# JakobHavtorn/benchmarking-lvms

Hardware: AMD Instinct MI355X
Metric: audio frames/sec training (VRNN, 16 kHz mu-law) (higher is better)
Workload: dtype f32

## Files before the change

### benchmarking-lvms_amd/csrc/pchain.h

```cpp
#pragma once
#include <algorithm>
#include <cstdlib>

#include "common.h"

namespace blvm {
namespace pchain {

constexpr unsigned SENTINEL = 0xFFFFFFFFu;
constexpr unsigned SPIN_LIMIT = 1u << 22;

typedef unsigned u32x4 __attribute__((ext_vector_type(4)));
typedef __amdgpu_buffer_rsrc_t rsrc_t;
constexpr int AUX_SC1 = 16;
#ifndef PCHAIN_POLL_AUX
#define PCHAIN_POLL_AUX AUX_SC1
#endif
#ifndef PCHAIN_STORE_AUX
#define PCHAIN_STORE_AUX AUX_SC1
#endif
__device__ __forceinline__ rsrc_t make_rsrc(const void* base) {
  const unsigned long long u = reinterpret_cast<unsigned long long>(base);
  const unsigned lo = (unsigned)__builtin_amdgcn_readfirstlane((int)(unsigned)u), hi = (unsigned)__builtin_amdgcn_readfirstlane((int)(unsigned)(u >> 32));
  return __builtin_amdgcn_make_buffer_rsrc(reinterpret_cast<void*>(((unsigned long long)hi << 32) | lo), 0, 0xFFFFFFFFu, 0x00020000);
}
__device__ __forceinline__ f32x4 ld_sc1_x4(rsrc_t r, unsigned byte_off) {
  return __builtin_bit_cast(f32x4, __builtin_amdgcn_raw_buffer_load_b128(r, (int)byte_off, 0, PCHAIN_POLL_AUX));
}
__device__ __forceinline__ float ld_sc1(rsrc_t r, unsigned byte_off) {
  return __builtin_bit_cast(float, __builtin_amdgcn_raw_buffer_load_b32(r, (int)byte_off, 0, PCHAIN_POLL_AUX));
}
__device__ __forceinline__ void st_sc1(rsrc_t r, unsigned byte_off, float v) {
  __builtin_amdgcn_raw_buffer_store_b32(__builtin_bit_cast(unsigned, v), r, (int)byte_off, 0, PCHAIN_STORE_AUX);
}

__device__ __forceinline__ bool is_sentinel(float x) { return __float_as_uint(x) == SENTINEL; }
__device__ __forceinline__ bool any_sentinel(const f32x4& v) {
  return is_sentinel(v[0]) | is_sentinel(v[1]) | is_sentinel(v[2]) | is_sentinel(v[3]);
}

struct Ctl {
  unsigned* dev;
  unsigned* host;
  unsigned epoch;
  __device__ __forceinline__ bool aborted() const { return __hip_atomic_load(dev, __ATOMIC_RELAXED, __HIP_MEMORY_SCOPE_AGENT) == epoch; }
  __device__ __forceinline__ void abort(unsigned code) const {
    if (__hip_atomic_exchange(dev, epoch, __ATOMIC_RELAXED, __HIP_MEMORY_SCOPE_AGENT) != epoch) {
      __hip_atomic_store(host + 1, code, __ATOMIC_RELAXED, __HIP_MEMORY_SCOPE_SYSTEM);
      __hip_atomic_fetch_add(host, 1u, __ATOMIC_RELAXED, __HIP_MEMORY_SCOPE_SYSTEM);
    }
  }
};

__device__ __forceinline__ bool spin_tick(unsigned& spins, const Ctl& ctl, unsigned code, bool& dead) {
  ++spins;
  if ((spins & 255u) == 0) {
    if (ctl.aborted()) { dead = true; return true; }
    if (spins >= SPIN_LIMIT) { ctl.abort(code); dead = true; return true; }
  }
  return false;
}

struct Poll {
  Ctl ctl;
  unsigned code;
  bool dead;
  int nap;
#ifdef PCHAIN_TPROF
  unsigned long long t_first = 0, t_ok = 0, t_end = 0, tp[8] = {0, 0, 0, 0, 0, 0, 0, 0};
  unsigned polls = 0;
#endif
  __device__ __forceinline__ void sleep() const {
    if (nap > 8) __builtin_amdgcn_s_sleep(32);
    else __builtin_amdgcn_s_sleep(1);
  }
};

struct MapSame { static constexpr int of(int) { return 0; } static constexpr bool sum = false; };
struct MapId { static constexpr int of(int g) { return g; } static constexpr bool sum = false; };
struct MapPairs { static constexpr int of(int g) { return g >> 1; } static constexpr bool sum = false; };
struct MapSum { static constexpr int of(int) { return 0; } static constexpr bool sum = true; };

struct NoMid {
  __device__ __forceinline__ void operator()() const {}
};

typedef short s16x4 __attribute__((ext_vector_type(4)));
typedef unsigned u32x2 __attribute__((ext_vector_type(2)));
typedef float f32x2_t __attribute__((ext_vector_type(2)));
typedef __bf16 bf16x2_t __attribute__((ext_vector_type(2)));
typedef _Float16 f16x2_t __attribute__((ext_vector_type(2)));
typedef _Float16 f16x4_t __attribute__((ext_vector_type(4)));
__device__ __forceinline__ unsigned pk_bf16(float a, float b) {
  return __builtin_bit_cast(unsigned, __builtin_convertvector((f32x2_t){a, b}, bf16x2_t));
}
template <int OT>
__device__ __forceinline__ unsigned pk16(float a, float b) {
  if constexpr (OT == OP_F16) return __builtin_bit_cast(unsigned, __builtin_convertvector((f32x2_t){a, b}, f16x2_t));
  else return pk_bf16(a, b);
}
template <int OT>
__device__ __forceinline__ f32x4 mfma16(s16x4 a, s16x4 b, f32x4 acc) {
  if constexpr (OT == OP_F16)
    return __builtin_amdgcn_mfma_f32_16x16x16f16(__builtin_bit_cast(f16x4_t, a), __builtin_bit_cast(f16x4_t, b), acc, 0, 0, 0);
  else return __builtin_amdgcn_mfma_f32_16x16x16bf16_1k(a, b, acc, 0, 0, 0);
}
template <int OT> struct WFrag { typedef u32x2 type; };
template <> struct WFrag<OP_F32> { typedef f32x4 type; };

template <int NW, int OT, int GA, int G, class AMap, int CH, class Mid>
__device__ __forceinline__ void mgemm_trip(const rsrc_t (&ar)[GA], unsigned aoff, const float* const (&ap)[GA], const char* const (&wp)[G], int kc,
                                           bool aok, bool polled, f32x4 (&acc)[G], Poll& pl, Mid& mid, bool& mid_pending) {
  constexpr int STEP = NW * 16;
  typedef typename WFrag<OT>::type wfrag;
  constexpr int ES = OT != OP_F32 ? 2 : 4;
  wfrag w[G][CH];
  f32x4 a[GA][CH];
#pragma unroll
  for (int u = 0; u < CH; ++u)
#pragma unroll
    for (int g = 0; g < G; ++g) w[g][u] = *reinterpret_cast<const wfrag*>(wp[g] + (size_t)ES * 16 * (size_t)(kc + u * STEP));
  if (!polled) {
#pragma unroll
// ... 303 lines not shown
  LinLate L;
  auto prefetch = [&]() {
    L = late();
    if (L.bias) e_bias = L.bias[col];
    if (L.gate) e_gate = L.gate[(size_t)rowc * L.ldgate + col];
    if (L.add && !L.add_polled) e_add = L.add[(size_t)rowc * L.ldadd + col];
  };
  f32x4 acc[1] = {{0.f, 0.f, 0.f, 0.f}};
  if (A2 != nullptr) {
    const float* const As[3] = {A, A2, A3};
    const float* const Ws[1] = {W};
    const int la[3] = {0, 0, 0}, cs[1] = {c0};
    tile_product<NW, OT, 3, 1, MapSum>(ws, As, la, true, r0, B, Ws, cs, K, acc, pl, prefetch, lda, w_width);
  } else {
    const float* const As[1] = {A};
    const float* const Ws[1] = {W};
    const int la[1] = {lda}, cs[1] = {c0};
    tile_product<NW, OT, 1, 1, MapSame>(ws, As, la, a_polled, r0, B, Ws, cs, K, acc, pl, prefetch, a_polled ? lda : 0, w_width);
  }
  float v[1];
  reduce_tiles<1, NW>(acc, red, v);
#ifdef PCHAIN_TPROF
  if (a_polled && pl.nap == 1) {
    const unsigned long long t3 = wall_clock64();
    pl.tp[0] += 1; pl.tp[1] += pl.t_first - t0; pl.tp[2] += pl.t_ok - pl.t_first; pl.tp[3] += t3 - pl.t_ok; pl.tp[4] += pl.polls;
    if (pl.t_end != 0) pl.tp[6] += t0 - pl.t_end;
  }
#endif
  if (threadIdx.x >= 256) return;
  if (L.add && L.add_polled) {
    const rsrc_t rs[1] = {make_rsrc(L.add)};
    const unsigned os[1] = {4u * ((unsigned)rowc * (unsigned)L.ldadd + (unsigned)col)};
    float ws[1];
    poll_words<1>(rs, os, ws, own, pl);
    e_add = ws[0];
  }
  if (!own) return;
  float x = v[0] + e_bias + e_add;
  if (L.relu) x = x > 0.f ? x : x * L.slope;
  if (L.gate) x = e_gate > 0.f ? x : x * L.slope;
  put(L.out, r0, c0, row, col, x);
#ifdef PCHAIN_TPROF
  if (a_polled && pl.nap == 1) { pl.t_end = wall_clock64(); }
#endif
}
template <int NW, int OT = OP_F32>
__device__ __forceinline__ void tile_lin(const float* A, int lda, bool a_polled, const float* W, int K, const float* bias,
                                         const float* add, int ldadd, bool add_polled, const float* gate, int ldgate, bool relu,
                                         float slope, const Out& out, int r0, int c0, int B, float* red, Poll& pl) {
  auto late = [&]() { return LinLate{bias, add, gate, ldadd, ldgate, add_polled, relu, slope, out}; };
  tile_lin_late<NW, OT>(A, lda, a_polled, W, K, late, r0, c0, B, red, pl);
}

struct HeadOut {
  float *mu_p, *sd_p, *mu_q, *sd_q, *raw_p, *raw_q, *muq_raw;
  Out z;
};
template <int NW, int OT = OP_F32, class WS = WMem>
__device__ __forceinline__ void tile_head(const float* P, const float* Q, bool polled, const float* Wp, const float* bp, const float* Wq,
                                          const float* bq, const float* eps, const HeadOut& o, int H, int Z, int residual, float beta,
                                          float inv_beta, float sd_eps, int r0, int c0, int B, float* red, Poll& pl, const WS& ws = WS()) {
  const int t = threadIdx.x & 255;
  const int row = r0 + (t >> 4), col = c0 + (t & 15);
  const bool own = threadIdx.x < 256 && row < B;
  const size_t oc = (size_t)(row < B ? row : r0) * Z + col;
  float b0 = 0.f, b1 = 0.f, b2 = 0.f, b3 = 0.f, e = 0.f;
  auto prefetch = [&]() { b0 = bp[col]; b1 = bp[Z + col]; b2 = bq[col]; b3 = bq[Z + col]; e = eps[oc]; };
  f32x4 acc[4];
#pragma unroll
  for (int g = 0; g < 4; ++g) acc[g] = (f32x4){0.f, 0.f, 0.f, 0.f};
  {
    const float* const As[2] = {P, Q};
    const float* const Ws[4] = {Wp, Wp, Wq, Wq};
    const int la[2] = {H, H}, cs[4] = {c0, Z + c0, c0, Z + c0};
    tile_product<NW, OT, 2, 4, MapPairs>(ws, As, la, polled, r0, B, Ws, cs, H, acc, pl, prefetch);
  }
  float v[4];
  reduce_tiles<4, NW>(acc, red, v);
  if (!own) return;
  const size_t oo = (size_t)row * Z + col;
  const float mp = v[0] + b0, rp = v[1] + b1, rq = v[3] + b3;
  float mq = v[2] + b2;
  const float sp = softplus_beta(rp, beta, inv_beta) + sd_eps;
  const float sq = softplus_beta(rq, beta, inv_beta) + sd_eps;
  if (o.muq_raw != nullptr) o.muq_raw[oo] = mq;
  float sqc = sq;
  if (residual == 1) {
    mq += mp;
  } else if (residual == 2) {
    const float pq = 1.f / (sq * sq), pp = 1.f / (sp * sp);
    const float var = 1.f / (pq + pp);
    mq = var * (mq * pq + mp * pp);
    sqc = sqrtf(var);
  } else if (residual == 3) {
    mq = mp;
    sqc = sp;
  }
  put(o.z, r0, c0, row, col, e * sqc + mq);
  o.mu_p[oo] = mp; o.sd_p[oo] = sp; o.mu_q[oo] = mq; o.sd_q[oo] = sqc;
  o.raw_p[oo] = rp; o.raw_q[oo] = rq;
}

template <int NW, int OT = OP_F32, class WS = WMem>
__device__ __forceinline__ void tile_gru(const float* X, int ldx, bool polled, const float* Wih, int K, const float* xg, const float* bih,
                                         const float* gh, const float* hprev, int ldh, int R, const Out& hnew, float* rg, float* ug, float* ng,
                                         int r0, int c0, int B, float* red, Poll& pl, const WS& ws = WS()) {
  const int t = threadIdx.x & 255;
  const int row = r0 + (t >> 4), col = c0 + (t & 15);
  const bool own = threadIdx.x < 256 && row < B;
  const int rowc = row < B ? row : r0;
  const size_t o3 = (size_t)rowc * 3 * R + col;
  const rsrc_t rgh = make_rsrc(gh), rhp = make_rsrc(hprev);
  const rsrc_t ps[4] = {rgh, rgh, rgh, rhp};
  const unsigned po[4] = {4u * (unsigned)o3, 4u * (unsigned)(o3 + R), 4u * (unsigned)(o3 + 2 * R), 4u * ((unsigned)rowc * (unsigned)ldh + (unsigned)col)};
  float w[4] = {0.f, 0.f, 0.f, 0.f}, x0 = 0.f, x1 = 0.f, x2 = 0.f;
  auto prefetch = [&]() {
#pragma unroll
    for (int i = 0; i < 4; ++i) w[i] = ld_sc1(ps[i], po[i]);
    x0 = (xg ? xg[o3] : 0.f) + (bih ? bih[col] : 0.f);
    x1 = (xg ? xg[o3 + R] : 0.f) + (bih ? bih[R + col] : 0.f);
    x2 = (xg ? xg[o3 + 2 * R] : 0.f) + (bih ? bih[2 * R + col] : 0.f);
  };
  f32x4 acc[3];
#pragma unroll
  for (int g = 0; g < 3; ++g) acc[g] = (f32x4){0.f, 0.f, 0.f, 0.f};
  {
    const float* const As[1] = {X};
    const float* const Ws[3] = {Wih, Wih, Wih};
    const int la[1] = {ldx}, cs[3] = {c0, R + c0, 2 * R + c0};
    tile_product<NW, OT, 1, 3, MapSame>(ws, As, la, polled, r0, B, Ws, cs, K, acc, pl, prefetch);
  }
  float v[3];
  reduce_tiles<3, NW>(acc, red, v);
  if (threadIdx.x >= 256) return;
  if (__any(own && (is_sentinel(w[0]) | is_sentinel(w[1]) | is_sentinel(w[2]) | is_sentinel(w[3])))) poll_words<4>(ps, po, w, own, pl);
  if (!own) return;
  const float r = sigmoidf_(v[0] + x0 + w[0]);
  const float u = sigmoidf_(v[1] + x1 + w[1]);
  const float n = tanhf(v[2] + x2 + r * w[2]);
  put(hnew, r0, c0, row, col, (1.f - u) * n + u * w[3]);
  const size_t o = (size_t)row * R + col;
  rg[o] = r; ug[o] = u; ng[o] = n;
}

struct DzIn {
  const float *mu_q, *sd_q, *mu_p, *sd_p, *eps, *raw_q, *raw_p, *muq_raw;
  const int32_t* x_sl;
  const float *c_raw, *c_fn;
  int t, stride, residual;
  float fn_floor, beta, sd_eps;
  bool has_gemm = true;
};
template <int NW, int OT = OP_F32, class WS = WMem>
__device__ __forceinline__ void tile_dz(const float* D, const float* WT, const float* D2, const float* WT2, bool polled, const float* dz_add,
                                        int ld_add, bool add_polled, const DzIn& a, const Out& dqh, const Out& dph, int H, int Z, int r0, int c0,
                                        int B, float* red, Poll& pl, const WS& ws = WS()) {
  const int t = threadIdx.x & 255;
  const int row = r0 + (t >> 4), col = c0 + (t & 15);
  const bool own = threadIdx.x < 256 && row < B;
  const int rowc = row < B ? row : r0;
  const size_t o = (size_t)rowc * Z + col;
  float mq = 0.f, sq = 1.f, mp = 0.f, sp = 1.f, e = 0.f, rq = 0.f, rp = 0.f, c_raw = 0.f, c_fn = 0.f, e_add = 0.f;
  auto prefetch = [&]() {
    mq = a.mu_q[o]; sq = a.sd_q[o]; mp = a.mu_p[o]; sp = a.sd_p[o]; e = a.eps[o]; rq = a.raw_q[o]; rp = a.raw_p[o];
    if (a.c_fn != nullptr || a.c_raw != nullptr) {
      const bool live = (long long)a.t * a.stride < a.x_sl[rowc];
      c_raw = (live && a.c_raw != nullptr) ? a.c_raw[rowc] : 0.f;
      c_fn = (live && a.c_fn != nullptr) ? a.c_fn[rowc] : 0.f;
    }
    if (dz_add != nullptr && !add_polled) e_add = dz_add[(size_t)rowc * ld_add + col];
  };
  float v[2] = {0.f, 0.f};
  if (a.has_gemm) {
    f32x4 acc[2];
    acc[0] = (f32x4){0.f, 0.f, 0.f, 0.f};
    acc[1] = (f32x4){0.f, 0.f, 0.f, 0.f};
    if (WS::products != 1 && D2 != nullptr) {
      if constexpr (WS::products != 1) {
        const float* const As[2] = {D, D2};
        const float* const Ws[2] = {WT, WT2};
        const int la[2] = {H, H}, cs[2] = {c0, c0};
        tile_product<NW, OT, 2, 2, MapId>(ws, As, la, polled, r0, B, Ws, cs, H, acc, pl, prefetch);
      }
    } else {
      if constexpr (WS::products != 2) {
        f32x4 a1[1] = {acc[0]};
        const float* const As[1] = {D};
        const float* const Ws[1] = {WT};
// ... 541 lines not shown
```

### benchmarking-lvms_amd/csrc/vrnn_static.h

```cpp
#pragma once
#include <algorithm>
#include <initializer_list>

#include "pchain.h"

namespace blvm {
namespace pchain {

struct LinkRange {
  int ct, wg0, nwg;
};
struct VrnnFwdDeal {
  int def_n, half, g;
  LinkRange hproj, prior, post, head, phi, gru;
};
inline VrnnFwdDeal vrnn_fwd_deal(int ctH, int ctZ, int ctR, int tl, int cus, bool shared) {
  VrnnFwdDeal d;
  d.def_n = shared ? 0 : range_for(3 * ctR * tl, std::min(cus / 4, 64));
  d.half = range_for(ctH * tl, (cus - d.def_n) / 2);
  d.g = 2 * d.half;
  const int wide = shared ? d.half : d.g;
  d.hproj = shared ? LinkRange{3 * ctR, d.half, d.half} : LinkRange{3 * ctR, d.g, d.def_n};
  d.prior = LinkRange{ctH, 0, d.half};
  d.post = LinkRange{ctH, d.half, d.half};
  d.head = LinkRange{ctZ, 0, range_for(ctZ * tl, wide)};
  d.phi = LinkRange{ctH, 0, range_for(ctH * tl, wide)};
  d.gru = LinkRange{ctR, 0, range_for(ctR * tl, d.g)};
  return d;
}
struct VrnnBwdDeal {
  int def_n, half, g, spare;
  bool split3;
  LinkRange grub, part[3], dphi, gb, wide_h, dz, prior, post;
};
inline VrnnBwdDeal vrnn_bwd_deal(int ctH, int ctZ, int ctR, int tl, int cus, bool shared, bool allow_split3) {
  VrnnBwdDeal d;
  d.def_n = shared ? 0 : range_for(ctR * tl, std::min(cus / 4, 64));
  d.half = range_for(ctH * tl, (cus - d.def_n) / 2);
  d.g = 2 * d.half;
  const int wide = shared ? d.half : d.g;
  d.spare = cus - d.g - d.def_n;
  d.split3 = !shared && d.spare >= 8 && d.half >= 8 && allow_split3;
  d.grub = LinkRange{ctR, 0, range_for(ctR * tl, d.g)};
  d.part[0] = LinkRange{ctH, 0, range_for(ctH * tl, d.half)};
  d.part[1] = LinkRange{ctH, d.half, range_for(ctH * tl, d.half)};
  d.part[2] = LinkRange{ctH, d.g + d.def_n, d.split3 ? range_for(ctH * tl, d.spare) : 0};
  d.dphi = LinkRange{ctH, 0, range_for(ctH * tl, wide)};
  d.gb = shared ? LinkRange{ctR, d.half, d.half} : LinkRange{ctR, d.g, d.def_n};
  d.wide_h = LinkRange{ctH, 0, range_for(ctH * tl, wide)};
  d.dz = LinkRange{ctZ, 0, range_for(ctZ * tl, wide)};
  d.prior = LinkRange{ctH, 0, d.half};
  d.post = LinkRange{ctH, d.half, d.half};
  return d;
}

constexpr std::initializer_list<int> kFwdResident = {1, 2, 3, 4, 5};
constexpr std::initializer_list<int> kBwdResident = {0, 1, 2, 3, 5, 6, 7, 8, 9};
inline bool one_tile_each(const Program& p, std::initializer_list<int> links) {
  for (int i : links)
    if (tiles_per_workgroup((p.B + 15) / 16, p.d[i].ct, p.d[i].nwg, p.xcd != 0) > 1) return false;
  return true;
}

}
}
```

### benchmarking-lvms_amd/csrc/vrnn_static.hip

```cpp
#include <algorithm>
#include <mutex>

#include "common.h"
#include "pchain.h"
#include "vrnn_static.h"

namespace blvm {
namespace {
using namespace pchain;

struct SPtr {
  float* base;
  int stride;
  __device__ __forceinline__ float* at(int s) const { return base + (long)s * stride; }
};

constexpr int kMaxTiles = 8;
__device__ __forceinline__ int tile_lanes(int w, int wg0, int nwg, int rt, int ct, bool xcd) {
  TileIter it(w, wg0, nwg, rt, ct, xcd);
  const int lane = threadIdx.x & 63;
  it.j += lane * it.step;
  return (lane < kMaxTiles && it.valid()) ? (it.r0() | (it.c() << 16)) : -1;
}
__device__ __forceinline__ int tile_count(int lanes) { return __popcll(__ballot(lanes >= 0)); }
// ... 109 lines not shown
  const int cs[1] = {tile_c0(tiles)};
  load_w<NW, OP_F32, 1, K / 256>(r.w, Ws, cs, ldw > 0 ? ldw : K);
}
template <int NW, int N, int K0, int K>
__device__ __forceinline__ void load_run(RunRes<N, K0, K>& r, const SeqArgs& q, int tiles, int nt) {
  load_lin<NW, K0>(r.first, q.W[0], K0, tiles, nt);
#pragma unroll
  for (int li = 1; li < N; ++li) load_lin<NW, K>(r.rest[li - 1], q.W[li], K, tiles, nt);
}
template <int NW>
__device__ __forceinline__ void load_head(Res<kH, 4>& r, const HeadArgs& q, int tiles, int nt) {
  if (nt == 0) return;
  const int c0 = tile_c0(tiles);
  const float* const Ws[4] = {q.Wp, q.Wp, q.Wq, q.Wq};
  const int cs[4] = {c0, q.Z + c0, c0, q.Z + c0};
  load_w<NW, OP_F32, 4, 1>(r.w, Ws, cs, kH);
}
template <int NW>
__device__ __forceinline__ void load_gru(Res<kH, 3>& r, const GruArgs& q, int tiles, int nt) {
  if (nt == 0) return;
  const int c0 = tile_c0(tiles);
  const float* const Ws[3] = {q.Wih, q.Wih, q.Wih};
  const int cs[3] = {c0, q.R + c0, 2 * q.R + c0};
  load_w<NW, OP_F32, 3, 1>(r.w, Ws, cs, kH);
}
template <int NW>
__device__ __forceinline__ void load_grub(Res<kH, 2>& r, const GrubArgs& q, int tiles, int nt) {
  if (nt == 0) return;
  const int c0 = tile_c0(tiles);
  const float* const Ws[2] = {q.W0, q.W1};
  const int cs[2] = {c0, c0};
  load_w<NW, OP_F32, 2, 1>(r.w, Ws, cs, kH);
}

template <int NW, int K, int FLAGS, class WS>
__device__ __forceinline__ void visit_lin(const LinArgs& q, const Deal& d, int s, int tiles, int nt, Walk& wk, const WS& ws) {
  if (nt == 0 || s < d.s_begin || s >= d.s_end) return;
  constexpr bool sum3 = (FLAGS & DF_A_SUM3) != 0;
  wk.at(d, s, (FLAGS & DF_GENTLE) != 0);
  const float* A = q.a.at(s);
  const float* A2 = sum3 ? q.a2.at(s) : nullptr;
  const float* A3 = sum3 ? q.a3.at(s) : nullptr;
  auto late = [&]() {
    return LinLate{q.bias, q.add.at(s), q.gate.at(s), q.ld1, q.ld2, (FLAGS & DF_ADD_POLLED) != 0, (FLAGS & DF_RELU) != 0, q.slope,
                   Out{q.orm.at(s), q.ld3, (FLAGS & DF_RM_SC1) != 0, q.o16.at(s), q.n16, q.o16b.at(s), q.n16b}};
  };
  for (int tk = 0; tk < (WS::resident ? 1 : nt); ++tk) {
    const int trc = __builtin_amdgcn_readlane(tiles, tk), tr0 = trc & 0xffff, tc0 = (trc >> 16) * 16;
    if constexpr ((FLAGS & DF_CANARY) != 0) canary_wait(A, tr0, K, wk.pl, q.ld0);
    tile_lin_late<NW, OP_F32>(A, q.ld0, true, q.W, K, late, tr0, tc0, wk.B, wk.red(), wk.pl, A2, A3, q.w_width, ws);
  }
}

template <int NW, int N, int K0, int K, bool GATED>
__device__ __forceinline__ void visit_run(const SeqArgs& q, const Deal& d, int s, int tiles, int nt, Walk& wk, const RunRes<N, K0, K>& rr) {
  if (nt == 0 || s < d.s_begin || s >= d.s_end) return;
  const int trc = __builtin_amdgcn_readlane(tiles, 0), tr0 = trc & 0xffff, tc0 = (trc >> 16) * 16;
  const float* A = q.a0.at(s);
#pragma unroll
  for (int li = 0; li < N; ++li) {
    wk.at(d, s, false, (unsigned)li);
    auto late = [&]() {
      const float* aux = q.aux[li].at(s);
      return LinLate{GATED ? nullptr : aux, li == 0 ? q.add0.at(s) : nullptr, GATED ? aux : nullptr, q.ldadd0, q.ldgate, false, !GATED, q.slope,
                     Out{q.orm[li].at(s), q.ld[li], false, q.o16[li].at(s), q.n16}};
    };
    if (li == 0) tile_lin_late<NW, OP_F32>(A, 0, true, q.W[li], K0, late, tr0, tc0, wk.B, wk.red(), wk.pl, nullptr, nullptr, 0, rr.first);
    else tile_lin_late<NW, OP_F32>(A, 0, true, q.W[li], K, late, tr0, tc0, wk.B, wk.red(), wk.pl, nullptr, nullptr, 0, rr.rest[li > 0 ? li - 1 : 0]);
    A = q.o16[li].at(s);
  }
}

template <int NW>
__device__ __forceinline__ void visit_head(const HeadArgs& q, const Deal& d, int s, int tiles, int nt, Walk& wk, const Res<kH, 4>& ws) {
  if (nt == 0 || s < d.s_begin || s >= d.s_end) return;
  wk.at(d, s, false);
  const HeadOut o{q.mu_p.at(s), q.sd_p.at(s), q.mu_q.at(s), q.sd_q.at(s), q.raw_p.at(s), q.raw_q.at(s), q.muq_raw.at(s),
                  Out{q.z.at(s), q.ld3, false, q.z16.at(s), q.n16, q.z16b.at(s), q.n16b}};
  const int trc = __builtin_amdgcn_readlane(tiles, 0);
  tile_head<NW, OP_F32>(q.P.at(s), q.Q.at(s), true, q.Wp, q.bp, q.Wq, q.bq, q.eps.at(s), o, kH, q.Z, q.residual, q.beta, q.inv_beta, q.sd_eps,
                        trc & 0xffff, (trc >> 16) * 16, wk.B, wk.red(), wk.pl, ws);
}

template <int NW>
__device__ __forceinline__ void visit_gru(const GruArgs& q, const Deal& d, int s, int tiles, int nt, Walk& wk, const Res<kH, 3>& ws) {
  if (nt == 0 || s < d.s_begin || s >= d.s_end) return;
  wk.at(d, s, false);
  const Out o{q.hrm.at(s), q.ld3, true, q.h16.at(s), q.n16, q.h16b.at(s), q.n16b};
  const int trc = __builtin_amdgcn_readlane(tiles, 0);
  tile_gru<NW, OP_F32>(q.X.at(s), 0, true, q.Wih, kH, q.xg.at(s), q.bih, q.gh.at(s), q.hprev.at(s), q.ld0, q.R, o, q.rg.at(s), q.ug.at(s), q.ng.at(s),
                       trc & 0xffff, (trc >> 16) * 16, wk.B, wk.red(), wk.pl, ws);
}

template <int NW>
__device__ __forceinline__ void visit_dz(const DzArgs& q, const Deal& d, int s, int tiles, int nt, Walk& wk, const Res<kH>& ws) {
  if (nt == 0 || s < d.s_begin || s >= d.s_end) return;
  wk.at(d, s, false);
  DzIn z;
  z.mu_q = q.mu_q.at(s); z.sd_q = q.sd_q.at(s); z.mu_p = q.mu_p.at(s); z.sd_p = q.sd_p.at(s); z.eps = q.eps.at(s); z.raw_q = q.raw_q.at(s);
  z.raw_p = q.raw_p.at(s); z.muq_raw = q.muq_raw.at(s);
  z.x_sl = q.x_sl; z.c_raw = q.c_raw; z.c_fn = q.c_fn;
  z.t = q.t0 - s; z.stride = q.stride; z.residual = q.residual;
  z.fn_floor = q.fn_floor; z.beta = q.beta; z.sd_eps = q.sd_eps;
  z.has_gemm = s >= q.first_gemm;
  const Out oq{q.dqh.at(s), q.ld3, false, q.dqh16.at(s), q.n16}, op{q.dph.at(s), q.ld3, false, q.dph16.at(s), q.n16};
  const int trc = __builtin_amdgcn_readlane(tiles, 0);
  tile_dz<NW, OP_F32>(q.D.at(s), q.WT, nullptr, nullptr, true, q.add.at(s), q.ld1, false, z, oq, op, kH, q.Z, trc & 0xffff, (trc >> 16) * 16, wk.B,
                      wk.red(), wk.pl, ws);
}

template <int NW>
__device__ __forceinline__ void visit_grub(const GrubArgs& q, const Deal& d, int s, int tiles, int nt, Walk& wk, const Res<kH, 2>& ws) {
  if (nt == 0 || s < d.s_begin || s >= d.s_end) return;
  wk.at(d, s, false);
  GrubIn g;
  g.D0 = q.D0.at(s); g.D1 = q.D1.at(s); g.W0 = q.W0; g.W1 = q.W1; g.g_in = q.g_in.at(s); g.g_add = q.g_add.at(s); g.ld_gadd = q.ld1;
  g.rg = q.rg.at(s); g.ug = q.ug.at(s); g.ng = q.ng.at(s); g.gh = q.gh.at(s); g.hprev = q.hprev.at(s); g.dd = q.dd.at(s); g.ldh = q.ld0;
  g.dgi = Out{q.dgi.at(s), q.ld3, false, q.dgi16.at(s), q.n16};
  g.dgh = Out{q.dgh.at(s), q.ld3, false, q.dgh16.at(s), q.n16};
  g.ga = q.ga.at(s); g.g_out = const_cast<float*>(q.g_out);
  g.has_gemm = s >= q.first_gemm; g.has_gates = s < q.end_gates; g.has_gin = s >= q.first_gin;
  const int trc = __builtin_amdgcn_readlane(tiles, 0);
  tile_grub<NW, OP_F32>(g, kH, q.R, trc & 0xffff, (trc >> 16) * 16, wk.B, wk.red(), wk.pl, ws);
}

template <class A>
__device__ __forceinline__ const A& kargs() {
  typedef const __attribute__((address_space(4))) char kchar;
  kchar* p = (kchar*)__builtin_amdgcn_kernarg_segment_ptr();
  asm volatile("" : "+s"(p));
  return *(const A*)p;
}

struct FwdArgs {
  LinArgs hproj;
  SeqArgs run[2];
  HeadArgs head;
  SeqArgs phi;
  GruArgs gru;
  Deal deal[6];
  int B, s0, S, xcd;
  Ctl ctl;
};
constexpr int kFwdProducts = 4, kBwdProducts = 2;

template <int NW, int HALF>
__device__ __forceinline__ void fwd_half(const FwdArgs& a, int w, int rt, bool xcd, Walk& wk) {
  const int t1 = tile_lanes(w, a.deal[1 + HALF].wg0, a.deal[1 + HALF].nwg, rt, a.deal[1 + HALF].ct, xcd), n1 = tile_count(t1);
  const int t3 = tile_lanes(w, a.deal[3].wg0, a.deal[3].nwg, rt, a.deal[3].ct, xcd), n3 = tile_count(t3);
  const int t4 = tile_lanes(w, a.deal[4].wg0, a.deal[4].nwg, rt, a.deal[4].ct, xcd), n4 = tile_count(t4);
  const int t5 = tile_lanes(w, a.deal[5].wg0, a.deal[5].nwg, rt, a.deal[5].ct, xcd), n5 = tile_count(t5);
  RunRes<3, kR, kH> run;
  Res<kH, 4> head;
  RunRes<4, kH, kH> phi;
  Res<kH, 3> gru;
  load_run<NW>(run, kargs<FwdArgs>().run[HALF], t1, n1);
  load_head<NW>(head, kargs<FwdArgs>().head, t3, n3);
  load_run<NW>(phi, kargs<FwdArgs>().phi, t4, n4);
  load_gru<NW>(gru, kargs<FwdArgs>().gru, t5, n5);
  for (int s = a.s0; s < a.S; ++s) {
    visit_run<NW, 3, kR, kH, false>(kargs<FwdArgs>().run[HALF], kargs<FwdArgs>().deal[1 + HALF], s, t1, n1, wk, run);
    visit_head<NW>(kargs<FwdArgs>().head, kargs<FwdArgs>().deal[3], s, t3, n3, wk, head);
    visit_run<NW, 4, kH, kH, false>(kargs<FwdArgs>().phi, kargs<FwdArgs>().deal[4], s, t4, n4, wk, phi);
    visit_gru<NW>(kargs<FwdArgs>().gru, kargs<FwdArgs>().deal[5], s, t5, n5, wk, gru);
  }
}

template <int NW>
__global__ __launch_bounds__(NW * 64, 1) void vrnn_static_fwd_kernel(FwdArgs a) {
  extern __shared__ __attribute__((aligned(16))) float lds_red[];
  const int w = blockIdx.x, rt = (a.B + 15) / 16;
  const bool xcd = a.xcd != 0;
  Walk wk{lds_red, lds_red + kFwdProducts * NW * 256, 0, a.B, Poll{a.ctl, 0u, false, 1}};
  if (w >= a.deal[0].wg0) {
    const int t0 = tile_lanes(w, a.deal[0].wg0, a.deal[0].nwg, rt, a.deal[0].ct, xcd), n0 = tile_count(t0);
    if (n0 == 0) return;
    for (int s = a.s0; s < a.S; ++s) visit_lin<NW, kR, DF_RM_SC1 | DF_GENTLE | DF_CANARY>(kargs<FwdArgs>().hproj, kargs<FwdArgs>().deal[0], s, t0, n0, wk, WMem());
    return;
  }
  if (w < a.deal[2].wg0) fwd_half<NW, 0>(a, w, rt, xcd, wk);
  else fwd_half<NW, 1>(a, w, rt, xcd, wk);
}

struct BwdArgs {
  GrubArgs grub;
  LinArgs part[3], gb, sum;
  SeqArgs phi;
  DzArgs dz;
  SeqArgs run[2];
  Deal deal[10];
  int B, s0, S, xcd;
  Ctl ctl;
};

template <int NW, int HALF>
__device__ __forceinline__ void bwd_half(const BwdArgs& a, int w, int rt, bool xcd, Walk& wk) {
  const int t0 = tile_lanes(w, a.deal[0].wg0, a.deal[0].nwg, rt, a.deal[0].ct, xcd), n0 = tile_count(t0);
  const int t1 = tile_lanes(w, a.deal[1 + HALF].wg0, a.deal[1 + HALF].nwg, rt, a.deal[1 + HALF].ct, xcd), n1 = tile_count(t1);
  const int t5 = tile_lanes(w, a.deal[5].wg0, a.deal[5].nwg, rt, a.deal[5].ct, xcd), n5 = tile_count(t5);
  const int t6 = tile_lanes(w, a.deal[6].wg0, a.deal[6].nwg, rt, a.deal[6].ct, xcd), n6 = tile_count(t6);
  const int t7 = tile_lanes(w, a.deal[7].wg0, a.deal[7].nwg, rt, a.deal[7].ct, xcd), n7 = tile_count(t7);
  const int t8 = tile_lanes(w, a.deal[8 + HALF].wg0, a.deal[8 + HALF].nwg, rt, a.deal[8 + HALF].ct, xcd), n8 = tile_count(t8);
  Res<kH, 2> grub;
  Res<kR> part;
  Res<kH> sum, dz;
  RunRes<2, kH, kH> phi;
  RunRes<3, 2 * kH, kH> run;
  load_grub<NW>(grub, kargs<BwdArgs>().grub, t0, n0);
  load_lin<NW, kR>(part, kargs<BwdArgs>().part[HALF].W, kargs<BwdArgs>().part[HALF].w_width, t1, n1);
  load_lin<NW, kH>(sum, kargs<BwdArgs>().sum.W, kH, t5, n5);
  load_run<NW>(phi, kargs<BwdArgs>().phi, t6, n6);
  load_lin<NW, kH>(dz, kargs<BwdArgs>().dz.WT, kH, t7, n7);
  load_run<NW>(run, kargs<BwdArgs>().run[HALF], t8, n8);
  for (int s = a.s0; s < a.S; ++s) {
    visit_grub<NW>(kargs<BwdArgs>().grub, kargs<BwdArgs>().deal[0], s, t0, n0, wk, grub);
    visit_lin<NW, kR, 0>(kargs<BwdArgs>().part[HALF], kargs<BwdArgs>().deal[1 + HALF], s, t1, n1, wk, part);
    visit_lin<NW, kH, DF_A_SUM3>(kargs<BwdArgs>().sum, kargs<BwdArgs>().deal[5], s, t5, n5, wk, sum);
    visit_run<NW, 2, kH, kH, true>(kargs<BwdArgs>().phi, kargs<BwdArgs>().deal[6], s, t6, n6, wk, phi);
    visit_dz<NW>(kargs<BwdArgs>().dz, kargs<BwdArgs>().deal[7], s, t7, n7, wk, dz);
    visit_run<NW, 3, 2 * kH, kH, true>(kargs<BwdArgs>().run[HALF], kargs<BwdArgs>().deal[8 + HALF], s, t8, n8, wk, run);
  }
}

template <int NW>
__global__ __launch_bounds__(NW * 64, 1) void vrnn_static_bwd_kernel(BwdArgs a) {
  extern __shared__ __attribute__((aligned(16))) float lds_red[];
  const int w = blockIdx.x, rt = (a.B + 15) / 16;
  const bool xcd = a.xcd != 0;
  Walk wk{lds_red, lds_red + kBwdProducts * NW * 256, 0, a.B, Poll{a.ctl, 0u, false, 1}};
  if (w >= a.deal[3].wg0) {
    const int t = tile_lanes(w, a.deal[3].wg0, a.deal[3].nwg, rt, a.deal[3].ct, xcd), n = tile_count(t);
    if (n == 0) return;
    Res<kR> part;
    load_lin<NW, kR>(part, kargs<BwdArgs>().part[2].W, kargs<BwdArgs>().part[2].w_width, t, n);
    for (int s = a.s0; s < a.S; ++s) visit_lin<NW, kR, 0>(kargs<BwdArgs>().part[2], kargs<BwdArgs>().deal[3], s, t, n, wk, part);
    return;
  }
  if (w >= a.deal[4].wg0) {
    const int t = tile_lanes(w, a.deal[4].wg0, a.deal[4].nwg, rt, a.deal[4].ct, xcd), n = tile_count(t);
    if (n == 0) return;
    for (int s = a.s0; s < a.S; ++s)
      visit_lin<NW, 3 * kR, DF_ADD_POLLED | DF_RM_SC1 | DF_GENTLE | DF_CANARY>(kargs<BwdArgs>().gb, kargs<BwdArgs>().deal[4], s, t, n, wk, WMem());
    return;
  }
  if (w < a.deal[2].wg0) bwd_half<NW, 0>(a, w, rt, xcd, wk);
  else bwd_half<NW, 1>(a, w, rt, xcd, wk);
}

bool int_strides(const Program& p) {
  for (long v : p.stride)
    if (v < -2147483647L || v > 2147483647L) return false;
  return true;
}
SPtr sptr(const Program& p, const Desc& d, int k) { return SPtr{const_cast<float*>(d.p[k]), (int)p.stride[d.sidx[k]]}; }

template <class Kern>
int static_go(Kern kernel, int slot, int grid, size_t lds, const char* what) {
  static std::mutex mu;
  static int attr_dev[3] = {-1, -1, -1}, occ[3] = {0, 0, 0};
  int dev = 0, cus = 0;
  BLVM_HIP(hipGetDevice(&dev));
  BLVM_HIP(hipDeviceGetAttribute(&cus, hipDeviceAttributeMultiprocessorCount, dev));
  {
    std::lock_guard<std::mutex> lock(mu);
    if (attr_dev[slot] != dev) {
      BLVM_HIP(hipFuncSetAttribute(reinterpret_cast<const void*>(kernel), hipFuncAttributeMaxDynamicSharedMemorySize, (int)lds));
      BLVM_HIP(hipOccupancyMaxActiveBlocksPerMultiprocessor(&occ[slot], kernel, 1024, lds));
      attr_dev[slot] = dev;
    }
    BLVM_REQUIRE((long)occ[slot] * cus >= grid, "%s: %d workgroups are not co-resident (%d per CU x %d CUs)", what, grid, occ[slot], cus);
  }
  return BLVM_OK;
}

int static_lin_chain_launch(const Program& p, hipStream_t stream, bool resident) {
  if (p.ndesc != 1 || p.ot != OP_F32 || p.rt_group != 1 || !int_strides(p)) return 1;
  const Desc& d = p.d[0];
  if (d.kind != K_LIN || d.flags != DF_RELU || d.f[LIN_F_SLOPE] != 0.f || (d.K != 256 && d.K != 512) || d.s_begin != 0 || d.s_end != p.S) return 1;
  if (d.ld[LIN_LD_A] != 0 || d.i[LIN_I_W_WIDTH] != 0 || d.p[LIN_ADD] || d.p[LIN_GATE] || d.p[LIN_O16B] || d.p[LIN_A2] || d.p[LIN_A3] || d.n16[N16_OUTB] != 0)
    return 1;
  const int rt = (p.B + 15) / 16;
  if (d.nwg <= 0 || (p.xcd && d.nwg % 8 != 0) || tiles_per_workgroup(rt, d.ct, d.nwg, p.xcd != 0) > (resident ? 1 : kMaxTiles)) return 1;
  LinChainArgs a{sptr(p, d, LIN_A), sptr(p, d, LIN_ORM), sptr(p, d, LIN_O16), d.p[LIN_W], d.p[LIN_BIAS], d.ld[LD_OUT], d.n16[N16_OUT], p.B, p.s_first, p.S,
                 d.wg0, d.nwg, d.ct, p.xcd, p.ctl};
  const int grid = d.wg0 + d.nwg;
  auto go = [&](auto kernel) -> int {
    BLVM_TRY(static_go(kernel, 2, grid, 0, "static_lin_chain"));
    hipLaunchKernelGGL(kernel, dim3(grid), dim3(1024), 0, stream, a);
    BLVM_CHECK_LAUNCH("static_lin_chain");
    return BLVM_OK;
  };
  if (resident) return d.K == 256 ? go(&static_lin_chain_kernel<16, 256, true>) : go(&static_lin_chain_kernel<16, 512, true>);
  return d.K == 256 ? go(&static_lin_chain_kernel<16, 256, false>) : go(&static_lin_chain_kernel<16, 512, false>);
}

int g_static = 1;
long g_static_launches = 0;
bool pchain_static_on() { return g_static != 0; }

SPtr sp(const Program& p, const Desc& d, int k) { return SPtr{const_cast<float*>(d.p[k]), d.p[k] ? (int)p.stride[d.sidx[k]] : 0}; }
Deal deal_of(const Desc& d, int idx) { return Deal{d.wg0, d.nwg, d.ct, d.s_begin, d.s_end, idx}; }
bool within(const Desc& d, int lo, int hi) { return d.wg0 >= lo && d.wg0 + d.nwg <= hi; }
bool few_tiles(const Program& p, const Desc& d) {
  if (d.nwg <= 0 || (p.xcd && d.nwg % 8 != 0)) return false;
  return tiles_per_workgroup((p.B + 15) / 16, d.ct, d.nwg, p.xcd != 0) <= kMaxTiles;
}
bool shaped(const Desc& d, int kind, int flags, int K) { return d.kind == kind && d.flags == flags && d.K == K; }
bool run(const Desc& d, int n, int K0) { return d.i[LINSEQ_I_N] == n && d.i[LINSEQ_I_K0] == K0; }

LinArgs lin_args(const Program& p, const Desc& d) {
  return LinArgs{sp(p, d, LIN_A), sp(p, d, LIN_A2), sp(p, d, LIN_A3), sp(p, d, LIN_ADD), sp(p, d, LIN_GATE), sp(p, d, LIN_ORM), sp(p, d, LIN_O16),
                 sp(p, d, LIN_O16B), d.p[LIN_W], d.p[LIN_BIAS], d.ld[LIN_LD_A], d.ld[LIN_LD_ADD], d.ld[LIN_LD_GATE], d.ld[LD_OUT], d.n16[N16_OUT], d.n16[N16_OUTB],
                 d.i[LIN_I_W_WIDTH], d.f[LIN_F_SLOPE]};
}
SeqArgs seq_args(const Program& p, const Desc& d) {
  SeqArgs q{};
  q.a0 = sp(p, d, LINSEQ_A0); q.add0 = sp(p, d, LINSEQ_ADD0);
  for (int i = 0; i < d.i[LINSEQ_I_N]; ++i) {
    q.W[i] = d.p[LINSEQ_W + i]; q.aux[i] = sp(p, d, LINSEQ_AUX + i); q.orm[i] = sp(p, d, LINSEQ_ORM + i); q.o16[i] = sp(p, d, LINSEQ_O16 + i);
    q.ld[i] = d.ld[LINSEQ_LD_ORM + i];
  }
  q.ldadd0 = d.i[LINSEQ_I_LD_ADD0]; q.ldgate = d.i[LINSEQ_I_LD_GATE]; q.n16 = d.n16[N16_OUT]; q.slope = d.f[LINSEQ_F_SLOPE];
  return q;
}

int vrnn_static_check(const Program& p, int ndesc, int products) {
  if (!pchain_static_on() || p.ndesc != ndesc || p.ot != OP_F32 || p.rt_group != 1 || p.s_first != 0 || p.B > 64) return 1;
  if (p.lds_products != products || !int_strides(p)) return 1;
  for (int i = 0; i < p.ndesc; ++i)
    if (!few_tiles(p, p.d[i])) return 1;
  return 0;
}

int vrnn_static_fwd(const Program& p, hipStream_t stream) {
  if (vrnn_static_check(p, 6, kFwdProducts)) return 1;
  const Desc* d = p.d;
  const int S = p.S;
  for (int i = 0; i < 6; ++i)
    if (d[i].s_begin != 0 || d[i].s_end != S) return 1;
  if (!shaped(d[0], K_LIN, DF_RM_SC1 | DF_GENTLE | DF_CANARY, kR) || !shaped(d[1], K_LINSEQ, DF_RELU, kH) || !shaped(d[2], K_LINSEQ, DF_RELU, kH) ||
      !shaped(d[3], K_HEAD, 0, kH) || !shaped(d[4], K_LINSEQ, DF_RELU, kH) || !shaped(d[5], K_GRU, 0, kH))
    return 1;
  if (!run(d[1], 3, kR) || !run(d[2], 3, kR) || !run(d[4], 4, 0)) return 1;
  if (!one_tile_each(p, kFwdResident)) return 1;
  const int half = d[2].wg0, gentle = d[0].wg0;
  if (d[1].wg0 != 0 || !within(d[1], 0, half) || !within(d[2], half, gentle) || d[0].nwg <= 0) return 1;
  for (int i = 3; i < 6; ++i)
    if (!within(d[i], 0, gentle)) return 1;
  FwdArgs a{};
  a.hproj = lin_args(p, d[0]);
  a.run[0] = seq_args(p, d[1]); a.run[1] = seq_args(p, d[2]); a.phi = seq_args(p, d[4]);
  const Desc &h = d[3], &g = d[5];
  a.head = HeadArgs{sp(p, h, HEAD_P16), sp(p, h, HEAD_Q16), sp(p, h, HEAD_EPS), sp(p, h, HEAD_MU_P), sp(p, h, HEAD_SD_P), sp(p, h, HEAD_MU_Q),
                    sp(p, h, HEAD_SD_Q), sp(p, h, HEAD_RAW_P), sp(p, h, HEAD_RAW_Q), sp(p, h, HEAD_MUQ_RAW), sp(p, h, HEAD_Z), sp(p, h, HEAD_Z16),
                    sp(p, h, HEAD_Z16B), h.p[HEAD_WP], h.p[HEAD_BP], h.p[HEAD_WQ], h.p[HEAD_BQ], h.ld[LD_OUT], h.n16[N16_OUT], h.n16[N16_OUTB],
                    h.i[HEAD_I_Z], h.i[HEAD_I_RESIDUAL], h.f[HEAD_F_BETA], h.f[HEAD_F_INV_BETA], h.f[HEAD_F_SD_EPS]};
  a.gru = GruArgs{sp(p, g, GRU_X16), sp(p, g, GRU_XG), sp(p, g, GRU_GH), sp(p, g, GRU_HPREV), sp(p, g, GRU_HRM), sp(p, g, GRU_H16), sp(p, g, GRU_H16B),
                  sp(p, g, GRU_RG), sp(p, g, GRU_UG), sp(p, g, GRU_NG), g.p[GRU_WIH], g.p[GRU_BIH], g.ld[GRU_LD_HPREV], g.ld[LD_OUT], g.n16[N16_OUT],
                  g.n16[N16_OUTB], g.i[GRU_I_R]};
  int grid = 0;
  for (int i = 0; i < 6; ++i) { a.deal[i] = deal_of(d[i], i); grid = std::max(grid, d[i].wg0 + d[i].nwg); }
  a.B = p.B; a.s0 = p.s_first; a.S = S; a.xcd = p.xcd; a.ctl = p.ctl;
  const size_t lds = sizeof(float) * 2 * kFwdProducts * 16 * 256;
  BLVM_TRY(static_go(&vrnn_static_fwd_kernel<16>, 0, grid, lds, "vrnn_static_fwd"));
  hipLaunchKernelGGL(vrnn_static_fwd_kernel<16>, dim3(grid), dim3(1024), lds, stream, a);
  BLVM_CHECK_LAUNCH("vrnn_static_fwd");
  ++g_static_launches;
  return BLVM_OK;
}

int vrnn_static_bwd(const Program& p, hipStream_t stream) {
  if (vrnn_static_check(p, 10, kBwdProducts)) return 1;
  const Desc* d = p.d;
  const int S = p.S;
  for (int i = 0; i < 10; ++i)
    if (d[i].s_begin != 0 || d[i].s_end != (i == 0 ? S : S - 1)) return 1;
  if (!shaped(d[0], K_GRUB, 0, kH) || !shaped(d[1], K_LIN, 0, kR) || !shaped(d[2], K_LIN, 0, kR) || !shaped(d[3], K_LIN, 0, kR) ||
      !shaped(d[4], K_LIN, DF_ADD_POLLED | DF_RM_SC1 | DF_GENTLE | DF_CANARY, 3 * kR) || !shaped(d[5], K_LIN, DF_A_SUM3, kH) ||
      !shaped(d[6], K_LINSEQ, DF_SEQ_GATE, kH) || !shaped(d[7], K_DZ, 0, kH) || !shaped(d[8], K_LINSEQ, DF_SEQ_GATE, kH) ||
      !shaped(d[9], K_LINSEQ, DF_SEQ_GATE, kH))
    return 1;
  if (!run(d[6], 2, 0) || !run(d[8], 3, 2 * kH) || !run(d[9], 3, 2 * kH)) return 1;
  if (!one_tile_each(p, kBwdResident) || d[7].p[DZ_D2_16] != nullptr) return 1;
  const int half = d[2].wg0, gentle = d[4].wg0, spare = d[3].wg0;
  if (!within(d[1], 0, half) || !within(d[8], 0, half) || !within(d[2], half, gentle) || !within(d[9], half, gentle) || !within(d[4], gentle, spare) ||
      d[3].nwg <= 0)
    return 1;
  for (int i : {0, 5, 6, 7})
    if (!within(d[i], 0, gentle)) return 1;
  BwdArgs a{};
  const Desc& g = d[0];
  a.grub = GrubArgs{sp(p, g, GRUB_D0_16), sp(p, g, GRUB_D1_16), sp(p, g, GRUB_G_IN), sp(p, g, GRUB_RG), sp(p, g, GRUB_UG), sp(p, g, GRUB_NG), sp(p, g, GRUB_GH),
                    sp(p, g, GRUB_HPREV), sp(p, g, GRUB_DD), sp(p, g, GRUB_DGI), sp(p, g, GRUB_DGI16), sp(p, g, GRUB_DGH), sp(p, g, GRUB_DGH16), sp(p, g, GRUB_GA),
                    sp(p, g, GRUB_G_ADD), g.p[GRUB_W0], g.p[GRUB_W1], g.p[GRUB_G_OUT], g.ld[GRUB_LD_H], g.ld[GRUB_LD_GADD], g.ld[LD_OUT], g.n16[N16_OUT],
                    g.i[GRUB_I_R], g.i[GRUB_I_GEMM_FROM], g.i[GRUB_I_GATES_TO], g.i[GRUB_I_GIN_FROM]};
  for (int k = 0; k < 3; ++k) a.part[k] = lin_args(p, d[1 + k]);
  a.gb = lin_args(p, d[4]); a.sum = lin_args(p, d[5]);
  a.phi = seq_args(p, d[6]); a.run[0] = seq_args(p, d[8]); a.run[1] = seq_args(p, d[9]);
  const Desc& z = d[7];
  a.dz = DzArgs{sp(p, z, DZ_D16), sp(p, z, DZ_ADD), sp(p, z, DZ_MU_Q), sp(p, z, DZ_SD_Q), sp(p, z, DZ_MU_P), sp(p, z, DZ_SD_P),
                sp(p, z, DZ_EPS), sp(p, z, DZ_RAW_Q), sp(p, z, DZ_RAW_P), sp(p, z, DZ_MUQ_RAW), sp(p, z, DZ_DQH), sp(p, z, DZ_DQH16), sp(p, z, DZ_DPH),
                sp(p, z, DZ_DPH16), z.p[DZ_WT], z.p[DZ_C_RAW], z.p[DZ_C_FN], reinterpret_cast<const int32_t*>(z.p[DZ_X_SL]), z.ld[DZ_LD_ADD],
                z.ld[LD_OUT], z.n16[N16_OUT], z.i[DZ_I_Z], z.i[DZ_I_RESIDUAL], z.i[DZ_I_STRIDE], z.i[DZ_I_T0], (int)z.f[DZ_F_GEMM_FROM], z.f[DZ_F_FN_FLOOR],
                z.f[DZ_F_BETA], z.f[DZ_F_SD_EPS]};
  int grid = 0;
  for (int i = 0; i < 10; ++i) { a.deal[i] = deal_of(d[i], i); grid = std::max(grid, d[i].wg0 + d[i].nwg); }
  a.B = p.B; a.s0 = p.s_first; a.S = S; a.xcd = p.xcd; a.ctl = p.ctl;
  const size_t lds = sizeof(float) * 2 * kBwdProducts * 16 * 256;
  BLVM_TRY(static_go(&vrnn_static_bwd_kernel<16>, 1, grid, lds, "vrnn_static_bwd"));
  hipLaunchKernelGGL(vrnn_static_bwd_kernel<16>, dim3(grid), dim3(1024), lds, stream, a);
  BLVM_CHECK_LAUNCH("vrnn_static_bwd");
  ++g_static_launches;
  return BLVM_OK;
}

}
// ... 42 lines not shown
```

Before: 80.41 million.

## Give hproj workgroups one register-resident 3-gate tile each in static forward

The forward persistent kernel's hidden-projection stage now assigns each workgroup a fixed (row tile, column) pair covering all three GRU gate columns. The Wih slices for those columns are loaded once into registers and reused across every timestep, replacing per-step memory weight reads through the generic lane dealer. This needs more workgroups (rt*ctR) to be co-resident, so the host checks occupancy and falls back if they do not fit. It also adds optional GRU-wait profiling counters that compile only under a debug macro.

```diff
diff --git a/benchmarking-lvms_amd/csrc/pchain.h b/benchmarking-lvms_amd/csrc/pchain.h
--- a/benchmarking-lvms_amd/csrc/pchain.h
+++ b/benchmarking-lvms_amd/csrc/pchain.h
@@ -69,6 +69,11 @@
 #ifdef PCHAIN_TPROF
   unsigned long long t_first = 0, t_ok = 0, t_end = 0, tp[8] = {0, 0, 0, 0, 0, 0, 0, 0};
   unsigned polls = 0;
+#endif
+#ifdef PCHAIN_GHWAIT
+  unsigned* gw_mark = nullptr;
+  unsigned gw_visit = 0, gw_tiles = 0, gw_waited = 0, gw_waves = 0;
+  unsigned long long gw_ticks = 0;
 #endif
   __device__ __forceinline__ void sleep() const {
     if (nap > 8) __builtin_amdgcn_s_sleep(32);
@@ -478,6 +483,40 @@
   tile_lin_late<NW, OT>(A, lda, a_polled, W, K, late, r0, c0, B, red, pl);
 }
 
+struct LinMultiLate {
+  const float* bias;
+  Out out;
+};
+template <int NW, int OT, int G, int NCH, class Late>
+__device__ __forceinline__ void tile_lin_multi(const float* A, int a_width, Late& late, int r0, int c0, int col_stride, int B, float* red, Poll& pl,
+                                               bool canary, const WRegs<OT, G, NCH>& ws) {
+  constexpr int K = NCH * 16 * NW;
+  const int t = threadIdx.x & 255;
+  const int row = r0 + (t >> 4), col = c0 + (t & 15);
+  const bool own = threadIdx.x < 256 && row < B;
+  float e_bias[G];
+  LinMultiLate L;
+  auto prefetch = [&]() {
+    L = late();
+#pragma unroll
+    for (int g = 0; g < G; ++g) e_bias[g] = L.bias ? L.bias[col + g * col_stride] : 0.f;
+  };
+  if (canary) canary_wait(A, r0, K, pl, a_width);
+  f32x4 acc[G];
+#pragma unroll
+  for (int g = 0; g < G; ++g) acc[g] = (f32x4){0.f, 0.f, 0.f, 0.f};
+  const float* const As[1] = {A};
+  product_regs<NW, OT, 1, G, MapSame, NCH, false>(As, r0, B, a_width > 0 ? a_width : K, ws.w, acc, pl, prefetch);
+  float v[G];
+  reduce_tiles<G, NW>(acc, red, v);
+  if (!own) return;
+#pragma unroll
+  for (int g = 0; g < G; ++g) {
+    const float x = v[g] + e_bias[g] + 0.f;
+    put(L.out, r0, c0 + g * col_stride, row, col + g * col_stride, x);
+  }
+}
+
 struct HeadOut {
   float *mu_p, *sd_p, *mu_q, *sd_q, *raw_p, *raw_q, *muq_raw;
   Out z;
@@ -559,7 +598,21 @@
   float v[3];
   reduce_tiles<3, NW>(acc, red, v);
   if (threadIdx.x >= 256) return;
+#ifdef PCHAIN_GHWAIT
+  ++pl.gw_visit;
+  pl.gw_tiles += threadIdx.x < 64;
+  if (__any(own && (is_sentinel(w[0]) | is_sentinel(w[1]) | is_sentinel(w[2]) | is_sentinel(w[3])))) {
+    const unsigned long long tw = wall_clock64();
+    poll_words<4>(ps, po, w, own, pl);
+    pl.gw_ticks += wall_clock64() - tw;
+    ++pl.gw_waves;
+    unsigned before = pl.gw_visit;
+    if (pl.gw_mark != nullptr && (threadIdx.x & 63) == 0) before = atomicMax(pl.gw_mark, pl.gw_visit);
+    pl.gw_waited += (unsigned)__builtin_amdgcn_readfirstlane((int)before) < pl.gw_visit;
+  }
+#else
   if (__any(own && (is_sentinel(w[0]) | is_sentinel(w[1]) | is_sentinel(w[2]) | is_sentinel(w[3])))) poll_words<4>(ps, po, w, own, pl);
+#endif
   if (!own) return;
   const float r = sigmoidf_(v[0] + x0 + w[0]);
   const float u = sigmoidf_(v[1] + x1 + w[1]);
diff --git a/benchmarking-lvms_amd/csrc/vrnn_static.h b/benchmarking-lvms_amd/csrc/vrnn_static.h
--- a/benchmarking-lvms_amd/csrc/vrnn_static.h
+++ b/benchmarking-lvms_amd/csrc/vrnn_static.h
@@ -28,6 +28,17 @@
   d.gru = LinkRange{ctR, 0, range_for(ctR * tl, d.g)};
   return d;
 }
+struct StaticHprojDeal {
+  int wg0, nwg, rt, R;
+  __host__ __device__ int grid() const { return wg0 + nwg; }
+  __host__ __device__ bool owns(int w) const { return w >= wg0 && w - wg0 < nwg; }
+  __host__ __device__ int r0(int w) const { return ((w - wg0) % rt) * 16; }
+  __host__ __device__ int c0(int w) const { return ((w - wg0) / rt) * 16; }
+  __host__ __device__ int col(int w, int gate) const { return gate * R + c0(w); }
+};
+inline StaticHprojDeal static_hproj_deal(int g, int rt, int ctR) { return StaticHprojDeal{g, rt * ctR, rt, 16 * ctR}; }
+inline bool static_hproj_fits(const StaticHprojDeal& d, int resident) { return d.nwg > 0 && d.grid() <= resident; }
+
 struct VrnnBwdDeal {
   int def_n, half, g, spare;
   bool split3;
diff --git a/benchmarking-lvms_amd/csrc/vrnn_static.hip b/benchmarking-lvms_amd/csrc/vrnn_static.hip
--- a/benchmarking-lvms_amd/csrc/vrnn_static.hip
+++ b/benchmarking-lvms_amd/csrc/vrnn_static.hip
@@ -185,6 +185,14 @@
   }
 }
 
+template <int NW>
+__device__ __forceinline__ void visit_hproj(const LinArgs& q, const Deal& d, int s, int r0, int c0, Walk& wk, const Res<kR, 3>& ws) {
+  if (s < d.s_begin || s >= d.s_end) return;
+  wk.at(d, s, true);
+  auto late = [&]() { return LinMultiLate{q.bias, Out{q.orm.at(s), q.ld3, true, nullptr, 0}}; };
+  tile_lin_multi<NW, OP_F32, 3>(q.a.at(s), q.ld0, late, r0, c0, kR, wk.B, wk.red(), wk.pl, true, ws);
+}
+
 template <int NW, int N, int K0, int K, bool GATED>
 __device__ __forceinline__ void visit_run(const SeqArgs& q, const Deal& d, int s, int tiles, int nt, Walk& wk, const RunRes<N, K0, K>& rr) {
   if (nt == 0 || s < d.s_begin || s >= d.s_end) return;
@@ -272,8 +280,12 @@
   SeqArgs phi;
   GruArgs gru;
   Deal deal[6];
+  StaticHprojDeal hp;
   int B, s0, S, xcd;
   Ctl ctl;
+#ifdef PCHAIN_GHWAIT
+  unsigned long long* prof;
+#endif
 };
 constexpr int kFwdProducts = 4, kBwdProducts = 2;
 
@@ -297,6 +309,12 @@
     visit_run<NW, 4, kH, kH, false>(kargs<FwdArgs>().phi, kargs<FwdArgs>().deal[4], s, t4, n4, wk, phi);
     visit_gru<NW>(kargs<FwdArgs>().gru, kargs<FwdArgs>().deal[5], s, t5, n5, wk, gru);
   }
+#ifdef PCHAIN_GHWAIT
+  if (a.prof != nullptr && (threadIdx.x & 63) == 0 && threadIdx.x < 256) {
+    atomicAdd(a.prof + 96, (unsigned long long)wk.pl.gw_tiles); atomicAdd(a.prof + 97, (unsigned long long)wk.pl.gw_waited);
+    atomicAdd(a.prof + 98, (unsigned long long)wk.pl.gw_waves); atomicAdd(a.prof + 99, wk.pl.gw_ticks);
+  }
+#endif
 }
 
 template <int NW>
@@ -305,10 +323,20 @@
   const int w = blockIdx.x, rt = (a.B + 15) / 16;
   const bool xcd = a.xcd != 0;
   Walk wk{lds_red, lds_red + kFwdProducts * NW * 256, 0, a.B, Poll{a.ctl, 0u, false, 1}};
-  if (w >= a.deal[0].wg0) {
-    const int t0 = tile_lanes(w, a.deal[0].wg0, a.deal[0].nwg, rt, a.deal[0].ct, xcd), n0 = tile_count(t0);
-    if (n0 == 0) return;
-    for (int s = a.s0; s < a.S; ++s) visit_lin<NW, kR, DF_RM_SC1 | DF_GENTLE | DF_CANARY>(kargs<FwdArgs>().hproj, kargs<FwdArgs>().deal[0], s, t0, n0, wk, WMem());
+#ifdef PCHAIN_GHWAIT
+  __shared__ unsigned gw_mark;
+  if (threadIdx.x == 0) gw_mark = 0;
+  __syncthreads();
+  wk.pl.gw_mark = &gw_mark;
+#endif
+  if (w >= a.hp.wg0) {
+    if (!a.hp.owns(w)) return;
+    const int r0 = a.hp.r0(w), c0 = a.hp.c0(w);
+    Res<kR, 3> hproj;
+    const float* const Ws[3] = {a.hproj.W, a.hproj.W, a.hproj.W};
+    const int cs[3] = {a.hp.col(w, 0), a.hp.col(w, 1), a.hp.col(w, 2)};
+    load_w<NW, OP_F32, 3, kR / 256>(hproj.w, Ws, cs, kR);
+    for (int s = a.s0; s < a.S; ++s) visit_hproj<NW>(kargs<FwdArgs>().hproj, kargs<FwdArgs>().deal[0], s, r0, c0, wk, hproj);
     return;
   }
   if (w < a.deal[2].wg0) fwd_half<NW, 0>(a, w, rt, xcd, wk);
@@ -388,21 +416,29 @@
 SPtr sptr(const Program& p, const Desc& d, int k) { return SPtr{const_cast<float*>(d.p[k]), (int)p.stride[d.sidx[k]]}; }
 
 template <class Kern>
-int static_go(Kern kernel, int slot, int grid, size_t lds, const char* what) {
+int static_resident(Kern kernel, int slot, size_t lds, long* resident, int* per_cu = nullptr, int* n_cus = nullptr) {
   static std::mutex mu;
   static int attr_dev[3] = {-1, -1, -1}, occ[3] = {0, 0, 0};
   int dev = 0, cus = 0;
   BLVM_HIP(hipGetDevice(&dev));
   BLVM_HIP(hipDeviceGetAttribute(&cus, hipDeviceAttributeMultiprocessorCount, dev));
-  {
-    std::lock_guard<std::mutex> lock(mu);
-    if (attr_dev[slot] != dev) {
-      BLVM_HIP(hipFuncSetAttribute(reinterpret_cast<const void*>(kernel), hipFuncAttributeMaxDynamicSharedMemorySize, (int)lds));
-      BLVM_HIP(hipOccupancyMaxActiveBlocksPerMultiprocessor(&occ[slot], kernel, 1024, lds));
-      attr_dev[slot] = dev;
-    }
-    BLVM_REQUIRE((long)occ[slot] * cus >= grid, "%s: %d workgroups are not co-resident (%d per CU x %d CUs)", what, grid, occ[slot], cus);
-  }
+  std::lock_guard<std::mutex> lock(mu);
+  if (attr_dev[slot] != dev) {
+    BLVM_HIP(hipFuncSetAttribute(reinterpret_cast<const void*>(kernel), hipFuncAttributeMaxDynamicSharedMemorySize, (int)lds));
+    BLVM_HIP(hipOccupancyMaxActiveBlocksPerMultiprocessor(&occ[slot], kernel, 1024, lds));
+    attr_dev[slot] = dev;
+  }
+  *resident = (long)occ[slot] * cus;
+  if (per_cu) *per_cu = occ[slot];
+  if (n_cus) *n_cus = cus;
+  return BLVM_OK;
+}
+template <class Kern>
+int static_go(Kern kernel, int slot, int grid, size_t lds, const char* what) {
+  long resident = 0;
+  int occ = 0, cus = 0;
+  BLVM_TRY(static_resident(kernel, slot, lds, &resident, &occ, &cus));
+  BLVM_REQUIRE(resident >= grid, "%s: %d workgroups are not co-resident (%d per CU x %d CUs)", what, grid, occ, cus);
   return BLVM_OK;
 }
 
@@ -476,6 +512,9 @@
     return 1;
   if (!run(d[1], 3, kR) || !run(d[2], 3, kR) || !run(d[4], 4, 0)) return 1;
   if (!one_tile_each(p, kFwdResident)) return 1;
+  const Desc& hp = d[0];
+  if (hp.p[LIN_ADD] || hp.p[LIN_GATE] || hp.p[LIN_O16] || hp.p[LIN_O16B] || hp.p[LIN_A2] || hp.p[LIN_A3] || hp.i[LIN_I_W_WIDTH] != 0) return 1;
+  if (hp.ct != 3 * (kR / 16) || hp.ld[LIN_LD_A] != 0 || !hp.p[LIN_ORM]) return 1;
   const int half = d[2].wg0, gentle = d[0].wg0;
   if (d[1].wg0 != 0 || !within(d[1], 0, half) || !within(d[2], half, gentle) || d[0].nwg <= 0) return 1;
   for (int i = 3; i < 6; ++i)
@@ -491,10 +530,17 @@
   a.gru = GruArgs{sp(p, g, GRU_X16), sp(p, g, GRU_XG), sp(p, g, GRU_GH), sp(p, g, GRU_HPREV), sp(p, g, GRU_HRM), sp(p, g, GRU_H16), sp(p, g, GRU_H16B),
                   sp(p, g, GRU_RG), sp(p, g, GRU_UG), sp(p, g, GRU_NG), g.p[GRU_WIH], g.p[GRU_BIH], g.ld[GRU_LD_HPREV], g.ld[LD_OUT], g.n16[N16_OUT],
                   g.n16[N16_OUTB], g.i[GRU_I_R]};
-  int grid = 0;
-  for (int i = 0; i < 6; ++i) { a.deal[i] = deal_of(d[i], i); grid = std::max(grid, d[i].wg0 + d[i].nwg); }
+  for (int i = 0; i < 6; ++i) a.deal[i] = deal_of(d[i], i);
   a.B = p.B; a.s0 = p.s_first; a.S = S; a.xcd = p.xcd; a.ctl = p.ctl;
   const size_t lds = sizeof(float) * 2 * kFwdProducts * 16 * 256;
+  a.hp = static_hproj_deal(gentle, (p.B + 15) / 16, kR / 16);
+  long resident = 0;
+  BLVM_TRY(static_resident(&vrnn_static_fwd_kernel<16>, 0, lds, &resident));
+  if (!static_hproj_fits(a.hp, (int)std::min<long>(resident, 1 << 30))) return 1;
+  const int grid = a.hp.grid();
+#ifdef PCHAIN_GHWAIT
+  a.prof = pchain_profile_buffer();
+#endif
   BLVM_TRY(static_go(&vrnn_static_fwd_kernel<16>, 0, grid, lds, "vrnn_static_fwd"));
   hipLaunchKernelGGL(vrnn_static_fwd_kernel<16>, dim3(grid), dim3(1024), lds, stream, a);
   BLVM_CHECK_LAUNCH("vrnn_static_fwd");
```

After: 81.70 million, median of 6. 1.02x the previous value.
